# HKUST-Aerial-Robotics/VINS-Mobile

Measured on AMD Instinct MI355X. Metric: VIO frames/sec (KLT+window solve), 640x480/150 feats/W=10, higher is better.
Workload: dtype f64 (solve) / u8+i32+f32 (KLT)

## Files before the change

### include/vio_amd.h

```cpp
#ifndef VIO_AMD_H
#define VIO_AMD_H

#include <stddef.h>
#include <stdint.h>

#ifdef __cplusplus
extern "C" {
#endif

#define VIO_ABI_VERSION 1

#define VIO_OK 0
#define VIO_EINVAL (-1)
#define VIO_ENODEV (-2)
#define VIO_ENOMEM (-3)
#define VIO_ECAP (-4)
#define VIO_ESTATE (-5)
#define VIO_ETIMEOUT (-6)

#define VIO_SIZE_POSE 7
#define VIO_SIZE_SPEEDBIAS 9
#define VIO_MAX_PRIOR_BLOCKS 96

typedef struct VioConfig {
// ... 98 lines not shown
int32_t vio_prior_capacity(int32_t window_size);

typedef struct vio_backend vio_backend_t;

int vio_backend_create(const VioConfig *cfg, int32_t max_batch, vio_backend_t **out);
int vio_backend_get_device(const vio_backend_t *be, int32_t *device);
void vio_backend_destroy(vio_backend_t *be);

int vio_preintegrate(const VioConfig *cfg, const double acc_0[3], const double gyr_0[3],
                     const double ba[3], const double bg[3], int32_t n,
                     const double *dt, const double *acc, const double *gyr,
                     VioPreintegration *out);

int vio_backend_solve_windows(vio_backend_t *be, VioWindow *windows, int32_t n,
                              int32_t buf_num, VioSolveStats *stats );

int vio_backend_reserve_priors(vio_backend_t *be, int32_t n_slots);

int vio_backend_upload(vio_backend_t *be, const VioWindow *windows, int32_t n);
int vio_backend_launch(vio_backend_t *be, void *stream);
int vio_backend_sync(vio_backend_t *be);
int vio_backend_download(vio_backend_t *be, VioWindow *windows, int32_t n, VioSolveStats *stats);
int vio_backend_kernel_ms(vio_backend_t *be, double *ms_avg, int32_t *launches);

#define VIO_N_STAGES 17
int vio_backend_set_profile(vio_backend_t *be, int32_t enable);
int vio_backend_stage_cycles(vio_backend_t *be, int32_t window, int64_t *cycles, int32_t n_stages);

typedef struct vio_frontend vio_frontend_t;

typedef struct VioObs {
  int32_t id;
  double x, y, z;
} VioObs;

typedef struct VioTrackViz {
  float *good_pts;
  double *track_len;
  int32_t cap;
  int32_t n;
} VioTrackViz;

int vio_frontend_create(const VioConfig *cfg, int32_t n_seq, vio_frontend_t **out);
int vio_frontend_get_device(const vio_frontend_t *fe, int32_t *device);
void vio_frontend_destroy(vio_frontend_t *fe);

// ... 469 lines not shown
```

### vins-mobile_amd/abi.py

```python
import ctypes as C
import os

import numpy as np

VIO_OK = 0
VIO_EINVAL, VIO_ENODEV, VIO_ENOMEM, VIO_ECAP, VIO_ESTATE, VIO_ETIMEOUT = -1, -2, -3, -4, -5, -6
VIO_MAX_PRIOR_BLOCKS = 96
VIO_MAX_TRACE = 64
VIO_INIT_BA_MAX_FRAMES = 16
VIO_BLOCK_POSE, VIO_BLOCK_SPEEDBIAS, VIO_BLOCK_EXPOSE = 0, 1, 2
VIO_MARGIN_OLD, VIO_MARGIN_SECOND_NEW, VIO_MARGIN_NONE = 0, 1, 2
STAGES = ["setup_imu", "setup_prior", "eval_prior", "eval_imu", "eval_proj", "scale", "schur", "rhs", "cholesky",
          "tri_solve", "quad_form", "dogleg", "cost_eval", "new2old", "marg_build", "marg_chol", "total",
          "p_zero", "p_fact", "p_gram", "p_feat", "c_potrf", "c_trsm", "imu_raw", "c_wait", "q_w", "backsolve",
          "c_ahead", "tr_vec", "m_prior", "m_imu", "m_fact", "m_gram", "d0", "d1", "d2", "d3", "d4", "d5",
          "v_gd", "v_dot", "v_step", "v_plus", "v_gmax", "v_rest", "b_init", "b_pose", "b_asp", "b_band", "b_gn",
          "e_head", "e_copy", "e_h0dx", "e_tail", "x0", "x1", "x2", "x3"]

_dp = C.POINTER(C.c_double)
_ip = C.POINTER(C.c_int32)


class VioConfig(C.Structure):
    _fields_ = [
# ... 388 lines not shown
    if not os.path.exists(PRODUCT_LIB):
        raise RuntimeError("HIP extension missing: %s (run __graft_entry__.build())" % PRODUCT_LIB)
    lib = C.CDLL(PRODUCT_LIB)
    vp = C.c_void_p
    lib.vio_version.restype = C.c_char_p
    lib.vio_config_default.argtypes = [C.POINTER(VioConfig)]
    lib.vio_prior_capacity.argtypes = [C.c_int32]
    lib.vio_prior_capacity.restype = C.c_int32
    lib.vio_backend_create.argtypes = [C.POINTER(VioConfig), C.c_int32, C.POINTER(vp)]
    lib.vio_backend_destroy.argtypes = [vp]
    lib.vio_backend_destroy.restype = None
    lib.vio_preintegrate.argtypes = [C.POINTER(VioConfig), _dp, _dp, _dp, _dp, C.c_int32, _dp, _dp, _dp,
                                     C.POINTER(VioPreintegration)]
    lib.vio_backend_solve_windows.argtypes = [vp, C.POINTER(VioWindow), C.c_int32, C.c_int32,
                                              C.POINTER(VioSolveStats)]
    lib.vio_backend_reserve_priors.argtypes = [vp, C.c_int32]
    lib.vio_backend_get_device.argtypes = [vp, C.POINTER(C.c_int32)]
    lib.vio_frontend_get_device.argtypes = [vp, C.POINTER(C.c_int32)]
    lib.vio_backend_upload.argtypes = [vp, C.POINTER(VioWindow), C.c_int32]
    lib.vio_backend_launch.argtypes = [vp, vp]
    lib.vio_backend_sync.argtypes = [vp]
    lib.vio_backend_download.argtypes = [vp, C.POINTER(VioWindow), C.c_int32, C.POINTER(VioSolveStats)]
    lib.vio_backend_kernel_ms.argtypes = [vp, _dp, _ip]
    u8p, fp = C.POINTER(C.c_uint8), C.POINTER(C.c_float)
    cfgp = C.POINTER(VioConfig)
    lib.vio_frontend_create.argtypes = [cfgp, C.c_int32, C.POINTER(vp)]
    lib.vio_frontend_destroy.argtypes = [vp]
    lib.vio_frontend_destroy.restype = None
    lib.vio_frontend_read_image.argtypes = [vp, C.c_int32, u8p, C.c_int32, C.c_int32, C.c_int32, C.c_double, C.c_int32,
                                            C.POINTER(VioObs), _ip, vp]
    lib.vio_frontend_read_images.argtypes = [vp, u8p, C.c_int32, C.c_int32, C.c_int32, _dp, C.c_int32,
                                             C.POINTER(VioObs), _ip]
    lib.vio_hip_runtime.argtypes = [C.c_char_p, C.c_int32, _ip]
    lib.vio_host_pool_width.argtypes = [_ip]
    lib.vio_frontend_submit_images.argtypes = [vp, u8p, C.c_int32, C.c_int32, C.c_int32, C.c_int32]
    lib.vio_frontend_submit_images_async.argtypes = [vp, u8p, C.c_int32, C.c_int32, C.c_int32, C.c_int32]
    lib.vio_frontend_collect.argtypes = [vp, C.POINTER(VioObs), _ip]
    lib.vio_host_register.argtypes = [vp, C.c_size_t]
    lib.vio_host_unregister.argtypes = [vp]
    lib.vio_frontend_upload_frames.argtypes = [vp, u8p, C.c_int32, C.c_int32, C.c_int32, C.c_int32]
    lib.vio_frontend_step_resident.argtypes = [vp, C.c_int32, C.c_int32, vp]
    lib.vio_frontend_sync.argtypes = [vp]
    lib.vio_frontend_kernel_ms.argtypes = [vp, _dp, _ip]
    lib.vio_frontend_get_state.argtypes = [vp, C.c_int32, fp, _ip, _ip, C.c_int32, _ip]
    lib.vio_frontend_get_pnp_points.argtypes = [vp, C.c_int32, fp, _ip, C.c_int32, _ip]
    lib.vio_frontend_lk_iterations.argtypes = [vp, C.c_int32, C.POINTER(C.c_uint64), C.POINTER(C.c_uint64), C.c_int32]
# ... 104 lines not shown
```

### vins-mobile_amd/backend.py

```python
import ctypes as C

import numpy as np

from . import abi


class WindowSolver:
    def __init__(self, cfg=None, max_batch=1024):
        self.lib = abi.load_product()
        self.cfg = cfg if cfg is not None else abi.default_config()
        self.max_batch = max_batch
        self._h = C.c_void_p()
        rc = self.lib.vio_backend_create(C.byref(self.cfg), max_batch, C.byref(self._h))
        if rc != abi.VIO_OK:
            raise RuntimeError("vio_backend_create failed rc=%d (a gfx950 device is required)" % rc)
        self._structs = None

    def close(self):
        if self._h:
            self.lib.vio_backend_destroy(self._h)
            self._h = C.c_void_p()

    def __del__(self):
        try:
# ... 3 lines not shown

    def _array(self, windows):
        arr = (abi.VioWindow * len(windows))()
        for i, w in enumerate(windows):
            w.fill_struct(arr[i])
        return arr

    @staticmethod
    def _check(rc, what):
        if rc != abi.VIO_OK:
            raise RuntimeError("%s failed rc=%d" % (what, rc))

    def solve(self, windows, buf_num=0):
        arr = self._array(windows)
        stats = (abi.VioSolveStats * len(windows))()
        self._check(self.lib.vio_backend_solve_windows(self._h, arr, len(windows), buf_num, stats), "solve_windows")
        return [abi.stats_to_dict(s) for s in stats]

    def device(self):
        d = C.c_int32(-1)
        self._check(self.lib.vio_backend_get_device(self._h, C.byref(d)), "get_device")
        return d.value

    def reserve_priors(self, n_slots):
        self._check(self.lib.vio_backend_reserve_priors(self._h, n_slots), "reserve_priors")

    def upload(self, windows):
        self._structs = self._array(windows)
        self._check(self.lib.vio_backend_upload(self._h, self._structs, len(windows)), "upload")

    def launch(self, stream=None):
        self._check(self.lib.vio_backend_launch(self._h, C.c_void_p(stream) if stream else None), "launch")

    def sync(self):
        self._check(self.lib.vio_backend_sync(self._h), "sync")

    def download(self, windows):
        arr = self._array(windows)
        stats = (abi.VioSolveStats * len(windows))()
        self._check(self.lib.vio_backend_download(self._h, arr, len(windows), stats), "download")
        return [abi.stats_to_dict(s) for s in stats]

    def set_profile(self, enable=True):
        self._check(self.lib.vio_backend_set_profile(self._h, 1 if enable else 0), "set_profile")

    def stage_cycles(self, window=0):
# ... 14 lines not shown
```

### vins-mobile_amd/csrc/solver_core.h

```cpp
#pragma once

#include <math.h>
#include <stdint.h>

#include <type_traits>

#include "solve_trace.h"
#include "vio_math.h"

#include "spmd.h"
#include "factors.h"
#include "mfma_tiles.h"

namespace vio {

constexpr int kBS = 15;
constexpr int kSS = kSB * kSB;
constexpr int kAW = 18;
constexpr int kAS = kSB * kAW;

struct WinView {
  int W, P, F, M, np, nblk, has_loop, loop_frame, marg_flag, max_iter;
  int prior_n, prior_nb;
  int Fpad;
// ... 992 lines not shown
  return total;
}


template <class WK>
VIO_DEV double feat_d2(const WK &w, int f) {
  return fmin(fmax(w.sf[f] * w.sf[f] * w.hff[f], 1e-6), 1e32);
}
template <class WK>
VIO_DEV double feat_d(const WK &w, int f) {
  return sqrt_f(feat_d2(w, f));
}
template <class WK>
VIO_DEV double feat_gd(const WK &w, int f) {
  return w.sf[f] * w.gf[f] * rsqrt_f(feat_d2(w, f));
}

template <class WK>
VIO_DEV double pose_gd(const WK &w, int i) {
  return w.sp[i] * w.gp[i] * rcp_f(w.dp[i]);
}

template <class WK>
VIO_DEV double quad_form_H(const Ctx &cx, const WinView &v, WK &w, cldsd vp, cldsd vf, bool prepared = false, bool w_part = true) {
  const int np = v.np, F = v.F, n6 = v.n6, P = v.P;
  if (!prepared) {
    VIO_PARFOR(f, F) w.tf[f] = 0.0;
    VIO_PARFOR(i, np) {
      const int f = i / kBS, c = i - f * kBS;
      const double u = w.sp[i] * vp[i];
      w.t1[i] = u;
      if (c < 6) w.xt[6 * f + c] = u;
    }
    VIO_SYNC();
  }
  int nparts, per;
  wt_parts((int)cx.nt, F, n6, nparts, per);
  if (w_part) VIO_PARFOR(q, F * nparts) {
    const int part = q / F, f = q - part * F;
    const int a0 = part * per, a1 = a0 + per < n6 ? a0 + per : n6;
    double x[kWStrip], sacc = 0;
    for (int b0 = a0; b0 < a1; b0 += kWStrip) {
      const int nb = a1 - b0 < kWStrip ? a1 - b0 : kWStrip;
      wt_strip_load(v.WTf + (size_t)f * v.n6cap + b0, 1, nb, x);
#pragma unroll
      for (int j = 0; j < kWStrip; j++) sacc += (j < nb ? x[j] : 0.0) * w.xt[b0 + (j < nb ? j : 0)];
    }
    VIO_ATOMIC_ADD(w.tf + f, sacc);
  }
  stamp(cx, ST_Q_W);
  double acc = 0;
  VIO_PARFOR(q, 4 * n6) {
    const int r = q >> 2, part = q & 3;
    auto row = w.App + tri_at(r, 0);
    double sacc = 0;
    for (int c = part; c < r; c += 4) sacc = fma(row[c], w.xt[c], sacc);
    sacc *= 2.0;
    if (part == 0) sacc = fma(row[r], w.xt[r], sacc);
    acc = fma(w.xt[r], sacc, acc);
  }
  VIO_PARFOR(q, P * kSB) {
// ... 14 lines not shown
    double s3 = 0, ar[kAW];
#pragma unroll
    for (int jj = 0; jj < kAW; jj++) ar[jj] = A[jj < aw ? jj : 0];
    VIO_SCHED_FENCE();
#pragma unroll
    for (int jj = 0; jj < kAW; jj++) s3 = fma(jj < aw ? ar[jj] : 0.0, w.xt[alo + (jj < aw ? jj : 0)], s3);
    acc = fma(ur, sacc + 2.0 * s3, acc);
  }
  VIO_PARFOR(q, kSB * v.nT) {
    const int c = q / v.nT, j0 = 16 * (q - c * v.nT);
    int kpr = -1;
    for (int k = 0; k < P; k++)
      if (w.sbr[2 * k + 1]) kpr = k;
    if (kpr < 0) continue;
    double xs[16], s3 = 0;
    const double *Ap = v.Apri + (size_t)c * v.jp + j0;
#pragma unroll
    for (int j = 0; j < 16; j++) xs[j] = Ap[j];
    VIO_SCHED_FENCE();
#pragma unroll
    for (int j = 0; j < 16; j++) s3 = fma(xs[j], j0 + j < n6 ? w.xt[j0 + j] : 0.0, s3);
    acc = fma(2.0 * w.t1[kBS * kpr + 6 + c], s3, acc);
  }
  if (w_part) VIO_SYNC();
  VIO_PARFOR(f, F) {
    const double u = w.sf[f] * vf[f];
    acc = fma(u, fma(w.hff[f], u, 2.0 * w.tf[f]), acc);
  }
  return block_sum(cx, acc);
}

template <class FT, class FR>
VIO_DEV void schur_ksplit5(const Ctx &cx, const double *Wf, int ldw, int n6, int F, cldsd einv, cldsd ge, FT flush_tile,
                           FR flush_rhs, cldsd up = nullptr, ldsd tq = nullptr) {
  constexpr int kT = 5;
  const int tid_ = VIO_TID(cx), wave = tid_ >> 6, lane = tid_ & 63, nw = cx.nt >> 6;
  const int li = lane & 15, kq = lane >> 4;
  const int ksteps = (F + 3) / 4;
  const int ksw = (ksteps + nw - 1) / nw;
  const int s_begin = wave * ksw, s_end = s_begin + ksw < ksteps ? s_begin + ksw : ksteps;
  v4d acc[kT * (kT + 1) / 2];
  double rp[kT];
#pragma unroll
  for (int q = 0; q < kT * (kT + 1) / 2; q++) acc[q] = v4d{0.0, 0.0, 0.0, 0.0};
#pragma unroll
  for (int t = 0; t < kT; t++) rp[t] = 0.0;
  double u5[kT];
#pragma unroll
  for (int t = 0; t < kT; t++) u5[t] = (tq && 16 * t + li < n6) ? up[16 * t + li] : 0.0;
  for (int s0 = s_begin; s0 < s_end; s0 += 5) {
    double wv[5][kT], ev[5], gv[5];
#pragma unroll
    for (int j = 0; j < 5; j++) {
      const int f = 4 * (s0 + j) + kq;
      const int fc = (s0 + j < s_end && f < F) ? f : 0;
      ev[j] = einv[fc], gv[j] = ge[fc];
#pragma unroll
      for (int t = 0; t < kT; t++) {
        const int col = 16 * t + li;
        wv[j][t] = Wf[(size_t)fc * ldw + (col < n6 ? col : 0)];
      }
    }
    __builtin_amdgcn_sched_barrier(0);
#pragma unroll
    for (int j = 0; j < 5; j++) {
      const int f = 4 * (s0 + j) + kq;
      const bool vf = s0 + j < s_end && f < F;
#pragma unroll
      for (int t = 0; t < kT; t++) {
        wv[j][t] = (vf && 16 * t + li < n6) ? wv[j][t] : 0.0;
        rp[t] = fma(wv[j][t], gv[j], rp[t]);
      }
      if (tq) {
        double pq = wv[j][0] * u5[0];
#pragma unroll
        for (int t = 1; t < kT; t++) pq = fma(wv[j][t], u5[t], pq);
        pq += dpp_move_f64<0x111, 0xf>(pq);
        pq += dpp_move_f64<0x112, 0xf>(pq);
        pq += dpp_move_f64<0x114, 0xf>(pq);
        pq += dpp_move_f64<0x118, 0xf>(pq);
        if (li == 15 && vf) tq[f] = pq;
      }
#pragma unroll
      for (int ti = 0; ti < kT; ti++) {
        const double a = wv[j][ti] * ev[j];
#pragma unroll
        for (int tj = 0; tj <= ti; tj++) acc[ti * (ti + 1) / 2 + tj] = mfma_f64(a, wv[j][tj], acc[ti * (ti + 1) / 2 + tj]);
      }
    }
  }
#pragma unroll
  for (int ti = 0; ti < kT; ti++)
#pragma unroll
    for (int tj = 0; tj <= ti; tj++) {
      const int bcol = 16 * tj + li;
#pragma unroll
      for (int r = 0; r < 4; r++) {
        const int arow = 16 * ti + kq + 4 * r;
        if (arow < n6 && bcol <= arow) flush_tile(arow, bcol, acc[ti * (ti + 1) / 2 + tj][r]);
      }
    }
#pragma unroll
  for (int t = 0; t < kT; t++) {
    const int a = 16 * t + li;
    if (a < n6 && rp[t] != 0.0) flush_rhs(a, rp[t]);
  }
}

VIO_DEV void schur_add(double *p, double v) { atomic_add_noret(p, v); }
#ifndef VIO_HOST_BUILD
VIO_DEV void schur_add(ldsd p, double v) { atomic_add(p, v); }
#endif

template <class FT, class FR>
VIO_DEV void schur_blocks(const Ctx &cx, const double *Wf, int ldw, int n6, int F, cldsd einv, cldsd ge, int share, int nshare, FT flush_el,
                          FR flush_rhs, cldsd up = nullptr, ldsd tq = nullptr) {
  const int T = (n6 + 15) / 16, NB = (T + 1) / 2, nblocks = NB * (NB + 1) / 2;
  const int tid_ = VIO_TID(cx), wave = tid_ >> 6, lane = tid_ & 63, nw = cx.nt >> 6;
  const int li = lane & 15, kq = lane >> 4;
  const int ksteps = (F + 3) / 4;
  constexpr int kChunk = 6;
  const int nchunks = (ksteps + kChunk - 1) / kChunk;
  int ksplit = 1;
  {
    const int waves = nshare * nw;
    int best = ((nblocks + waves - 1) / waves) * nchunks;
    for (int k = 2; k <= 4; k++) {
      const int cost = ((nblocks * k + waves - 1) / waves) * ((nchunks + k - 1) / k);
      if (cost < best) best = cost, ksplit = k;
    }
  }
  const int ks_part = (nchunks + ksplit - 1) / ksplit * kChunk;
  for (int u = share * nw + wave; u < nblocks * ksplit; u += nshare * nw) {
    const int p = u / ksplit, part = u - p * ksplit;
    const int s_lo = part * ks_part, s_hi = s_lo + ks_part < ksteps ? s_lo + ks_part : ksteps;
    int I = 0;
    while ((I + 1) * (I + 2) / 2 <= p) I++;
    const int J = p - I * (I + 1) / 2;
    const bool diag = I == J;
    const int ta[2] = {2 * I, 2 * I + 1}, tb[2] = {2 * J, 2 * J + 1};
    bool va[2], vb[2];
    const double *pa[2], *pb[2];
#pragma unroll
    for (int q = 0; q < 2; q++) {
      va[q] = ta[q] < T && 16 * ta[q] + li < n6, vb[q] = tb[q] < T && 16 * tb[q] + li < n6;
      pa[q] = Wf + (va[q] ? 16 * ta[q] + li : 0), pb[q] = Wf + (vb[q] ? 16 * tb[q] + li : 0);
    }
    v4d c00 = {0.0, 0.0, 0.0, 0.0}, c01 = c00, c10 = c00, c11 = c00;
    double rp[2] = {0.0, 0.0};
    const bool do_tq = diag && tq != nullptr;
    double u2[2] = {0.0, 0.0};
    if (do_tq) {
#pragma unroll
      for (int q = 0; q < 2; q++) u2[q] = va[q] ? up[16 * ta[q] + li] : 0.0;
    }
    for (int s0 = s_lo; s0 < s_hi; s0 += kChunk) {
      double av[2][kChunk], bv[2][kChunk], ev[kChunk], gv[kChunk];
#pragma unroll
      for (int j = 0; j < kChunk; j++) {
        const int f = 4 * (s0 + j) + kq;
        const size_t fo = (size_t)((f < F && s0 + j < s_hi) ? f : 0) * ldw;
        av[0][j] = pa[0][fo], av[1][j] = pa[1][fo], bv[0][j] = pb[0][fo], bv[1][j] = pb[1][fo];
        ev[j] = einv[(f < F && s0 + j < s_hi) ? f : 0];
        gv[j] = diag ? ge[(f < F && s0 + j < s_hi) ? f : 0] : 0.0;
      }
      VIO_SCHED_FENCE();
#pragma unroll
      for (int j = 0; j < kChunk; j++) {
        const int f = 4 * (s0 + j) + kq;
        const bool vf = f < F && s0 + j < s_hi;
        double pq = 0.0;
#pragma unroll
        for (int q = 0; q < 2; q++) {
          const double a_raw = (va[q] && vf) ? av[q][j] : 0.0;
          if (diag) rp[q] = fma(a_raw, gv[j], rp[q]);
          if (do_tq) pq = fma(a_raw, u2[q], pq);
          av[q][j] = a_raw * ev[j], bv[q][j] = (vb[q] && vf) ? bv[q][j] : 0.0;
        }
        if (do_tq) {
          pq += dpp_move_f64<0x111, 0xf>(pq);
          pq += dpp_move_f64<0x112, 0xf>(pq);
          pq += dpp_move_f64<0x114, 0xf>(pq);
          pq += dpp_move_f64<0x118, 0xf>(pq);
          if (li == 15 && vf) VIO_ATOMIC_ADD(tq + f, pq);
        }
      }
#pragma unroll
      for (int j = 0; j < kChunk; j++) {
        c00 = mfma_f64(av[0][j], bv[0][j], c00), c10 = mfma_f64(av[1][j], bv[0][j], c10), c11 = mfma_f64(av[1][j], bv[1][j], c11);
        if (!diag) c01 = mfma_f64(av[0][j], bv[1][j], c01);
      }
    }
    auto flush = [&](int tr, int tc, const v4d &acc) {
      const int bcol = 16 * tc + li;
#pragma unroll
      for (int r = 0; r < 4; r++) {
        const int arow = 16 * tr + kq + 4 * r;
        if (tr < T && tc < T && arow < n6 && bcol < n6 && bcol <= arow) flush_el(arow, bcol, acc[r], ksplit > 1);
      }
    };
    flush(ta[0], tb[0], c00), flush(ta[1], tb[0], c10), flush(ta[1], tb[1], c11);
    if (!diag) flush(ta[0], tb[1], c01);
    if (diag) {
#pragma unroll
      for (int q = 0; q < 2; q++)
        if (va[q] && rp[q] != 0.0) flush_rhs(16 * ta[q] + li, rp[q]);
    }
  }
}

template <class WK>
VIO_DEV void schur_general(const Ctx &cx, const WinView &v, WK &w, int share, int nshare, ldsd tq = nullptr) {
  const int n6 = v.n6, F = v.F;
  schur_blocks(
      cx, v.WTf, v.n6cap, n6, F, w.einv, w.tf, share, nshare,
      [&](int arow, int bcol, double val, bool parts) {
        if (parts) schur_add(w.App + tri_at(arow, bcol), -val);
        else w.App[tri_at(arow, bcol)] -= val;
      },
      [&](int a, double val) { schur_add(w.App + tri_at(n6, a), -val); },
      w.xt, tq);
  stamp(cx, ST_SCHUR);
}

template <class WK>
VIO_DEV bool build_reduced_system(const Ctx &cx, const WinView &v, WK &w, double mu, ldsd tq = nullptr) {
  const int np = v.np, F = v.F;
  stamp(cx, ST_TR_VEC);
  VIO_PARFOR(f, F) {
    const double isf = rcp_f(w.sf[f]);
    const double e = w.hff[f] + mu * (feat_d2(w, f) * isf * isf);
    const double ei = rcp_f(e);
    w.einv[f] = ei;
    w.tf[f] = w.gf[f] * ei;
    if (!(e > 0.0)) w.flag[0] = 1;
  }
  const bool tq_general = tq != nullptr && ((v.n6 + 15) >> 4) > 5;
  if (tq_general) VIO_PARFOR(f, F) tq[f] = 0.0;
  VIO_PARFOR(i, np) {
    const int f = i / kBS, c = i - f * kBS;
    const double cc = w.dp[i] * rcp_f(w.sp[i]);
    if (c < 6) {
      w.App[tri_at(6 * f + c, 6 * f + c)] += mu * cc * cc;
      w.App[tri_at(v.n6, 6 * f + c)] = w.gp[i];
    } else {
      w.Dss[f * kSS + (c - 6) * (kSB + 1)] += mu * cc * cc;
    }
  }
  VIO_SYNC();
  stamp(cx, ST_SCALE);
  const int n6 = v.n6;
  {
    const int T = (n6 + 15) / 16, npairs = T * (T + 1) / 2;
    const int tid_ = VIO_TID(cx), wave = tid_ >> 6, lane = tid_ & 63, nw = cx.nt >> 6;
    const int li = lane & 15, kq = lane >> 4;
    const int ksteps = (F + 3) / 4;
    constexpr int kT = 5;
    if (T <= kT) {
      schur_ksplit5(cx, v.WTf, v.n6cap, n6, F, w.einv, w.tf,
                    [&](int arow, int bcol, double val) { VIO_ATOMIC_ADD(w.App + tri_at(arow, bcol), -val); },
                    [&](int a, double val) { VIO_ATOMIC_ADD(w.App + tri_at(n6, a), -val); }, w.xt, tq);
    } else {
#ifndef VIO_HOST_BUILD
      if (cx.coop > 1) {
        const CoopLayout L = CoopLayout::make(v.Pcap, v.Fcap, v.nblk_cap);
        VIO_PARFOR(f, F) v.coop[L.o_einv + f] = w.einv[f], v.coop[L.o_tf + f] = w.tf[f];
        if (tq) VIO_PARFOR(q, 16 * T) v.coop[L.o_pose + q] = w.xt[q];
        coop_post(cx, v, COOP_SCHUR);
        schur_general(cx, v, w, 0, cx.coop, tq);
        coop_wait_helpers(cx, v);
        if (tq) {
          VIO_SYNC();
          for (int m = 1; m < cx.coop; m++) {
            const double *pr = v.coop + L.o_part + (size_t)(m - 1) * L.part;
            VIO_PARFOR(f, F) tq[f] += pr[L.p_f + f];
          }
        }
      } else
#endif
        schur_general(cx, v, w, 0, 1, tq);
    }
  }
  VIO_SYNC();
  stamp(cx, ST_RHS);
  (void)np;
  return w.flag[0] == 0;
}


template <class WK>
VIO_DEV void band_step(const Ctx &cx, const WinView &v, WK &w, int k, int fail_flag, int lane_) {
  const int lane = VIO_OPAQUE(lane_), li = lane & 15, kq = lane >> 4;
  ldsd D = w.Dss + k * kSS;
  ldsd ldk = w.ldinv + kSB * k;
  const bool good = potrf9_inv_wave(D, w.Css + (k + 1 <= v.W ? k + 1 : k) * kSS, k < v.W, ldk, lane);
  if (!good && lane == 0) w.flag[fail_flag] = 1;
  stamp(cx, ST_D3);
  if (k >= 1) {
    __builtin_amdgcn_fence(__ATOMIC_RELEASE, "wavefront");
    __builtin_amdgcn_wave_barrier();
    __builtin_amdgcn_fence(__ATOMIC_ACQUIRE, "wavefront");
    ldsd C = w.Css + k * kSS;
    double a[3], b[4];
// ... 936 lines not shown
};

template <bool REGS, int NW, class WK, class VP, class WP>
VIO_DEV void minimize(const Ctx &cx, const WinView &v, WK &w_whole, const VP &fresh, const WP &fresh_work) {
  WK &w = w_whole;
  const int np = v.np, F = v.F;
  const SolveTrace trace{v.stats_d, v.stats_i};
  auto grad_max_norm = [&]() { return gradient_max_norm(cx, fresh(), w); };

  double x_cost = evaluate(cx, fresh(), w, w.xpose, w.xsb, w.xfeat, true, false);
  double x_norm = -1.0;
  VIO_PARFOR(f, F) w.sf[f] = rcp_f(1.0 + sqrt_f(w.hff[f]));
  VIO_SYNC();
  double gmax = grad_max_norm();
  double radius = 1e4, mu = 1e-8;
  const double min_mu = 1e-8, max_mu = 1.0, mu_inc = 10.0;
  bool reuse = false, last_ok = true, have_factor = false;
  double dogleg_step_norm = 0, alpha = 0;
  int it = 0, n_ok = 1, n_bad = 0, invalid_run = 0, termination = 0, recorded = 1;
  StepEvaluator ev = StepEvaluator::at(x_cost);
  double min_rec = x_cost;
  if (cx.tid == 0) trace.record(0, x_cost, radius, 0, 0, gmax, true, true);
  if (cx.tid == 0) trace.initial(x_cost);
  double gd_sq = 0, mu_used = mu, qf_cauchy = 0, qf_part = 0;
  bool qf_pending = false;
  bool relin = false, relin_reuse = false, rec_pending = false;
  int rec_it = 0;
  double rec_step_norm = 0, rec_rho = 0;

  while (true) {
    WK w_iter = fresh_work();
    WK &w = w_iter;
    if (relin) {
      evaluate(cx, fresh(), w, w.xpose, w.xsb, w.xfeat, true, true, relin_reuse);
      if (rec_pending) {
        gmax = grad_max_norm();
        if (cx.tid == 0) trace.record(rec_it, x_cost, radius, rec_step_norm, rec_rho, gmax, true, true);
        stamp(cx, ST_V_GMAX);
      }
      relin = relin_reuse = rec_pending = false;
    }
    if (it >= v.max_iter) break;
    if (last_ok && gmax <= 1e-10) { termination = 1; break; }
    if (radius <= 1e-32) { termination = 1; break; }
    it++;
    bool solver_ok = true;
    if (!reuse) {
      reuse = true;
      ldsd park = w.park;
      if (cx.tid == 0) {
        park[0] = x_cost, park[1] = x_norm, park[2] = gmax, park[3] = radius, park[4] = dogleg_step_norm, park[5] = ev.minimum_cost;
        park[6] = ev.current_cost, park[7] = ev.reference_cost, park[8] = ev.candidate_cost;
        park[9] = ev.accumulated_reference_model_cost_change, park[10] = ev.accumulated_candidate_model_cost_change, park[11] = min_rec;
        ldsi pi = reinterpret_cast<ldsi>(park + 12);
        pi[0] = it, pi[1] = n_ok, pi[2] = n_bad, pi[3] = invalid_run, pi[4] = termination, pi[5] = recorded, pi[6] = last_ok ? 1 : 0;
      }
      {
        double part = 0;
        VIO_PARFOR(i, np) {
          const int f = i / kBS, c = i - f * kBS;
          const double g = pose_gd(w, i), a = g * rcp_f(w.dp[i]), u = w.sp[i] * a;
          part += g * g;
          w.t2[i] = a, w.t1[i] = u;
          if (c < 6) w.xt[6 * f + c] = u;
        }
        VIO_PARFOR(f, F) {
          const double d2 = feat_d2(w, f), sg = w.sf[f] * w.gf[f], g = sg * rsqrt_f(d2);
          part += g * g;
          w.stf[f] = sg * rcp_f(d2), w.tf[f] = 0.0;
        }
        gd_sq = block_sum(cx, part);
      }
      stamp(cx, ST_V_GD);
      const bool fuse_qw = true;
      const double qf_h0 = quad_form_H(cx, fresh(), w, w.t2, w.stf, true, !fuse_qw);
      stamp(cx, ST_QUADFORM);
      solver_ok = false;
      bool first_try = true;
      while (mu < max_mu) {
        if (!first_try) {
          evaluate(cx, fresh(), w, w.xpose, w.xsb, w.xfeat, true, true);
          if (fuse_qw) {
            VIO_PARFOR(i, np) {
              const int f = i / kBS, c = i - f * kBS;
              const double u = w.sp[i] * (pose_gd(w, i) * rcp_f(w.dp[i]));
              w.t1[i] = u;
              if (c < 6) w.xt[6 * f + c] = u;
            }
          }
        }
        first_try = false;
        if (cx.tid == 0) w.flag[0] = 0, w.flag[1] = 0, w.flag[2] = 0, w.flag[3] = 0;
        VIO_PARFOR(k, v.P) w.ready[k] = 0;
        VIO_SYNC();
        bool ok = build_reduced_system(cx, fresh(), w, mu, fuse_qw ? w.cfeat : nullptr);
        if (ok) {
          if constexpr (REGS) ok = factor_band_regs<kPanelTiles, NW>(cx, fresh(), w);
          else ok = factor_band_lds(cx, fresh(), w);
        }
        if (ok) ok = factor_poses(cx, fresh(), w);
        stamp(cx, ST_CHOL);
        if (ok) {
          backsolve(cx, fresh(), w);
          double bad = 0;
          VIO_PARFOR(f, F) {
            double y = (w.tf[f] - w.gnf[f] * w.einv[f]) * rcp_f(w.sf[f]);
            w.gnf[f] = -feat_d(w, f) * y;
            if (!isfinite(y)) bad = 1;
          }
          VIO_PARFOR(i, np) {
            double y = w.t1[i] * rcp_f(w.sp[i]);
            w.gnp[i] = -w.dp[i] * y;
            if (!isfinite(y)) bad = 1;
          }
          if (block_max(cx, bad) > 0) ok = false;
          stamp(cx, ST_TRISOLVE);
        }
        if (ok) { solver_ok = true; mu_used = mu; have_factor = true; break; }
        mu *= mu_inc;
      }
      {
        VIO_SYNC();
        x_cost = park[0], x_norm = park[1], gmax = park[2], radius = park[3], dogleg_step_norm = park[4], ev.minimum_cost = park[5];
        ev.current_cost = park[6], ev.reference_cost = park[7], ev.candidate_cost = park[8];
        ev.accumulated_reference_model_cost_change = park[9], ev.accumulated_candidate_model_cost_change = park[10], min_rec = park[11];
        ldsi pi = reinterpret_cast<ldsi>(park + 12);
        it = pi[0], n_ok = pi[1], n_bad = pi[2], invalid_run = pi[3], termination = pi[4], recorded = pi[5], last_ok = pi[6] != 0;
      }
      if (solver_ok) {
        qf_part = qf_h0, qf_pending = fuse_qw;
        if (!fuse_qw) {
          qf_cauchy = qf_h0 + mu_used * gd_sq;
          alpha = gd_sq / qf_h0;
        }
        stamp(cx, ST_DOGLEG);
      }
    }
    (void)have_factor;
    bool step_valid = false;
    double model_cost_change = 0;
    if (solver_ok) {
      double p1 = 0, p2 = 0, p3 = 0;
      VIO_PARFOR(i, np) p1 += w.gnp[i] * w.gnp[i], p2 += pose_gd(w, i) * w.gnp[i];
      VIO_PARFOR(f, F) {
        p1 += w.gnf[f] * w.gnf[f], p2 += feat_gd(w, f) * w.gnf[f];
        if (qf_pending) p3 += 2.0 * (w.sf[f] * w.sf[f] * w.gf[f] * rcp_f(feat_d2(w, f))) * w.cfeat[f];
      }
      block_sum3(cx, p1, p2, p3);
      stamp(cx, ST_V_DOT);
      if (qf_pending) {
        const double qf_h = qf_part + p3;
        qf_cauchy = qf_h + mu_used * gd_sq;
        alpha = gd_sq / qf_h;
        qf_pending = false;
      }
      double gnn2 = p1, gdot = p2;
      double gradient_norm = sqrt(gd_sq), gauss_newton_norm = sqrt(gnn2);
      double ca, cb;
      bool need_norm = false;
      if (gauss_newton_norm <= radius) {
        ca = 0, cb = 1, dogleg_step_norm = gauss_newton_norm;
      } else if (gradient_norm * alpha >= radius) {
        ca = -(radius / gradient_norm), cb = 0, dogleg_step_norm = radius;
      } else {
        double b_dot_a = -alpha * gdot;
        double a_squared_norm = pow(alpha * gradient_norm, 2.0);
        double b_minus_a_squared_norm = a_squared_norm - 2 * b_dot_a + pow(gauss_newton_norm, 2);
        double c = b_dot_a - a_squared_norm;
        double d = sqrt(c * c + b_minus_a_squared_norm * (pow(radius, 2.0) - a_squared_norm));
        double beta = (c <= 0) ? (d - c) / b_minus_a_squared_norm : (radius * radius - a_squared_norm) / (d + c);
        ca = -alpha * (1.0 - beta), cb = beta;
        need_norm = true;
      }
      VIO_PARFOR(i, np) {
        const double s_ = ca * pose_gd(w, i) + cb * w.gnp[i];
        w.t2[i] = s_ * rcp_f(w.dp[i]) * w.sp[i];
      }
// ... 129 lines not shown
      }
      VIO_PARFOR(q, nFr * 36) w.ppd[q] = 0.0;
      VIO_SYNC();
      VIO_PARFOR(i, nFr + 1) {
        const bool is_ex = i == nFr;
        double R[9];
        if (is_ex) qtoR(Quat{w.ex[3], w.ex[4], w.ex[5], w.ex[6]}, R);
        else qtoR(Quat{w.xpose[7 * i + 3], w.xpose[7 * i + 4], w.xpose[7 * i + 5], w.xpose[7 * i + 6]}, R);
        auto dst = w.rot + 9 * (is_ex ? v.P + 1 : i);
        for (int k = 0; k < 9; k++) dst[k] = R[k];
      }
      VIO_SYNC();
      const double cost = block_sum(cx, projections_jac(cx, v, w, w.xpose, w.xfeat, true, cx.member, cx.coop, false));
      ldsd whv[6] = {w.cfeat, w.stf, w.gnf, w.tf, w.ef, w.einv};
      VIO_PARFOR(q, np) part[L.p_gp + q] = w.gp[q];
      VIO_PARFOR(q, nFr * 36) part[L.p_ppd + q] = w.ppd[q];
      VIO_PARFOR(f, F) {
        part[L.p_f + f] = w.hff[f], part[L.p_f + fs + f] = w.gf[f];
#pragma unroll
        for (int c = 0; c < 6; c++) part[L.p_f + (2 + c) * fs + f] = whv[c][f];
      }
      if (cx.tid == 0) part[L.p_cost] = cost;
    } else if (cmd == COOP_SCHUR) {
      VIO_PARFOR(f, F) w.einv[f] = v.coop[L.o_einv + f], w.tf[f] = v.coop[L.o_tf + f], w.cfeat[f] = 0.0;
      VIO_PARFOR(q, 16 * ((v.n6 + 15) >> 4)) w.xt[q] = v.coop[L.o_pose + q];
      VIO_SYNC();
      schur_general(cx, v, w, cx.member, cx.coop, w.cfeat);
      VIO_SYNC();
      VIO_PARFOR(f, F) part[L.p_f + f] = w.cfeat[f];
    } else if (cmd == COOP_SYRK) {
      band_syrk_share(cx, v, w, cx.member, cx.coop);
    } else {
      break;
    }
    coop_done(cx, v);
  }
}
#endif

template <bool REGS, int NW, class WK, class VP, class WP>
VIO_DEV void solve_window(const Ctx &cx, const WinView &v, WK &w, const VP &fresh, const WP &fresh_work) {
  const int P = v.P, F = v.F;
  VIO_PARFOR(q, P * 7) w.xpose[q] = v.pose0[q];
  VIO_PARFOR(q, P * 9) w.xsb[q] = v.sb0[q];
  VIO_PARFOR(q, F) w.xfeat[q] = v.feat0[q];
  VIO_PARFOR(q, 7) w.ex[q] = v.ex[q];
  if (v.has_loop) VIO_PARFOR(q, 7) w.xpose[7 * P + q] = v.pose0[7 * v.loop_frame + q];
  VIO_PARFOR(q, v.nblk * kBS) w.t1[q] = 0.0, w.t2[q] = 0.0;
  if (cx.tid == 0) w.flag[0] = w.flag[1] = w.flag[2] = w.flag[3] = 0;
  init_band_reach(cx, v, w);
  VIO_SYNC();
  if (cx.prof && cx.tid == cx.prof_tid) {
// ... 71 lines not shown
```

### vins-mobile_amd/csrc/vio_backend.hip

```cpp
#include <hip/hip_runtime.h>

#include <stdio.h>
#include <stdlib.h>

#include <algorithm>
#include <memory>
#include <vector>

#include <chrono>

#include "batch.h"
#include "vio_pool.h"
#include "vio_device.h"
#include "marg_core.h"
#include "vio_window_variants.h"
#include "vio_amd.h"

using namespace vio;

namespace {

using vio_wk::kThreadsGlb;
using vio_wk::kThreadsLds;
constexpr size_t kLdsLimit = vio::kLdsBytes;
// ... 31 lines not shown

struct vio_backend {
  VioConfig cfg;
  std::unique_ptr<vio_resident> res;
  int peers = 2;
  int device = -1;
  int max_batch = 0;
  hipStream_t stream = nullptr;
  LaunchTimer timer;
  int n = 0;
  bool uploaded = false;
  hipStream_t last_stream = nullptr;
  hipEvent_t upload_done = nullptr;
  bool lds_matrix = true;
  int n_lds = 0, n_glb = 0;
  BatchDims d_lds, d_glb;
  size_t lds_bytes_glb = 0;
  DevBuf<int> d_order;
  HostVec<int> h_order;
  bool profile = false;
  size_t lds_bytes = 0;
  int n_cus = 256;
  bool static_w = false;
  bool coop_ok = false;
  DevBuf<long long> d_prof;
  HostBatch hb;
  BatchPtrs B;
  MargPtrs MP;
  DevBuf<unsigned char> d_in;
  DevBuf<int> d_stats_i, d_m_ints;
  DevBuf<double> d_scratch,
      d_hm, d_out_pose, d_out_sb, d_out_feat, d_raw_pose, d_raw_sb, d_raw_feat, d_out_loop, d_stats_d, d_m_x0, d_m_J,
      d_m_r, d_m_scratch;
  int st_n = 0, st_ncap = 0;
  DevBuf<double> d_st_x0[2], d_st_J[2], d_st_r[2];
  std::vector<unsigned char> st_bank;
  std::vector<int> slot_of;
  DevBuf<PriorTab> d_ptab;
  HostVec<PriorTab> h_ptab;
  bool host_prior_in = true, host_prior_out = true, slots_advanced = false;
  HostVec<double> h_out_pose, h_out_sb, h_out_feat, h_raw_pose, h_raw_sb, h_raw_feat, h_out_loop, h_stats_d, h_m_x0,
      h_m_J, h_m_r;
  HostVec<int> h_stats_i, h_m_ints;
  ~vio_backend();
};

// ... 367 lines not shown
  VIO_ON_DEVICE_OF(be);
  hipStream_t st = stream ? (hipStream_t)stream : be->stream;
  if (st != be->stream && be->upload_done) HIP_OK(hipStreamWaitEvent(st, be->upload_done, 0));
  be->last_stream = st;
  if (poison()) {
    HIP_OK(hipMemsetAsync(be->d_scratch.p, 0xff, be->d_scratch.n * sizeof(double), st));
    HIP_OK(hipMemsetAsync(be->d_hm.p, 0xff, be->d_hm.n * sizeof(double), st));
    HIP_OK(hipMemsetAsync(be->d_out_pose.p, 0xff, be->d_out_pose.n * sizeof(double), st));
    HIP_OK(hipMemsetAsync(be->d_stats_d.p, 0xff, be->d_stats_d.n * sizeof(double), st));
    HIP_OK(hipFuncSetAttribute((const void *)poison_lds_kernel, hipFuncAttributeMaxDynamicSharedMemorySize, (int)kLdsLimit));
    hipLaunchKernelGGL(poison_lds_kernel, dim3(2048), dim3(1024), kLdsLimit, st, (int)(kLdsLimit / sizeof(double)));
  }
  {
    const int rct = be->timer.begin(st);
    if (rct != VIO_OK) return rct;
  }
  if (be->n_lds > 0) {
    BatchPtrs Bl = be->B;
    Bl.d = be->d_lds, Bl.order = be->d_order.p;
    int variant = be->d_lds.lds_asp ? 0 : 1;
    if (be->static_w) variant += 3;
    vio_wk::variant(variant, be->MP.prof != nullptr).launch(be->n_lds, be->lds_bytes, st, Bl, be->MP);
  }
  if (be->n_glb > 0) {
    BatchPtrs Bg = be->B;
    Bg.d = be->d_glb, Bg.order = be->d_order.p + be->n_lds;
    int coop = 1;
    if (be->coop_ok && !be->MP.prof && be->lds_bytes_glb > kLdsHalf) {
      const int forced = vio::env_int("VIO_AMD_COOP", 0);
      const int cus = be->n_cus / std::max(1, be->peers);
      const int groups = (be->n_glb + 7) / 8;
      const bool four = groups * 8 * 4 <= cus && (be->d_glb.Wcap >= 24 || groups * 8 * 8 <= cus);
      coop = four ? 4 : groups * 8 * 2 <= cus ? 2 : 1;
      if (forced >= 1 && forced <= vio::kCoopMax && groups * 8 * forced <= cus) coop = forced;
      if (coop > 1) {
        int per_cu = 0;
        if (hipOccupancyMaxActiveBlocksPerMultiprocessor(&per_cu, vio_wk::variant(2, false).fn,
                                                         kThreadsGlb, be->lds_bytes_glb) != hipSuccess ||
            (long long)per_cu * cus < (long long)groups * 8 * coop)
          coop = 1;
      }
    }
    Bg.coop = coop, Bg.n_launch = be->n_glb;
    {
      const int spin = vio::env_int("VIO_AMD_COOP_SPIN", 0);
      Bg.coop_spin = spin > 0 ? (unsigned)spin : vio::kCoopSpinLimit;
      Bg.coop_fault = vio::env_flag("VIO_AMD_COOP_FAULT") ? 1 : 0;
    }
    int grid = be->n_glb;
    if (coop > 1) {
      grid = (be->n_glb + 7) / 8 * 8 * coop;
      HIP_OK(hipMemset2DAsync(be->d_scratch.p + be->B.s.s_coop, be->B.s.scratch * sizeof(double), 0, 32, (size_t)be->B.n, st));
    }
    vio_wk::variant(2, be->MP.prof != nullptr).launch(grid, be->lds_bytes_glb, st, Bg, be->MP);
  }
  HIP_OK(hipGetLastError());
  return be->timer.end(st);
}

int vio_backend_sync(vio_backend_t *be) {
  if (!be) return VIO_EINVAL;
  VIO_ON_DEVICE_OF(be);
  HIP_OK(hipDeviceSynchronize());
  return VIO_OK;
}

int vio_backend_kernel_ms(vio_backend_t *be, double *ms_avg, int32_t *launches) {
  if (!be || !ms_avg || !launches) return VIO_EINVAL;
  VIO_ON_DEVICE_OF(be);
  HIP_OK(hipDeviceSynchronize());
  return be->timer.drain(ms_avg, launches);
}

int vio_backend_set_profile(vio_backend_t *be, int32_t enable) {
  if (!be) return VIO_EINVAL;
  be->profile = enable != 0;
  be->uploaded = false;
  return VIO_OK;
}

int vio_backend_stage_cycles(vio_backend_t *be, int32_t window, int64_t *cycles, int32_t n_stages) {
  if (!be || !cycles || n_stages < 1) return VIO_EINVAL;
  if (!be->uploaded || !be->profile || window < 0 || window >= be->n) return VIO_ESTATE;
  VIO_ON_DEVICE_OF(be);
  HIP_OK(hipDeviceSynchronize());
  long long tmp[ST_COUNT];
  HIP_OK(hipMemcpy(tmp, be->d_prof.p + (size_t)window * ST_COUNT, sizeof(tmp), hipMemcpyDeviceToHost));
  for (int i = 0; i < n_stages; i++) cycles[i] = i < ST_COUNT ? (int64_t)tmp[i] : 0;
  return VIO_OK;
}

static int backend_download_impl(vio_backend_t *be, VioWindow *windows, int32_t n, VioSolveStats *stats);

int vio_backend_download(vio_backend_t *be, VioWindow *windows, int32_t n, VioSolveStats *stats) {
// ... 100 lines not shown
```

Before: 192,100.

## Compute Cauchy quad form lazily only when GN step exceeds radius

Removes the fused accumulation of the H-quadratic-form partials from the Schur complement kernels and the eager gradient/quad-form pass before each solve. Instead, the steepest-descent norm and quad form are computed only when the Gauss-Newton step falls outside the trust region. This path re-evaluates the residuals and stashes and restores the GN step in scratch. It also adds a query for the cooperative launch width. This saves work in the common in-radius case and lightens the Schur inner loops, at the cost of an extra evaluate call when dogleg is needed.

```diff
diff --git a/include/vio_amd.h b/include/vio_amd.h
--- a/include/vio_amd.h
+++ b/include/vio_amd.h
@@ -144,6 +144,7 @@
 int vio_backend_sync(vio_backend_t *be);
 int vio_backend_download(vio_backend_t *be, VioWindow *windows, int32_t n, VioSolveStats *stats);
 int vio_backend_kernel_ms(vio_backend_t *be, double *ms_avg, int32_t *launches);
+int vio_backend_coop_width(const vio_backend_t *be, int32_t *width);
 
 #define VIO_N_STAGES 17
 int vio_backend_set_profile(vio_backend_t *be, int32_t enable);
diff --git a/vins-mobile_amd/abi.py b/vins-mobile_amd/abi.py
--- a/vins-mobile_amd/abi.py
+++ b/vins-mobile_amd/abi.py
@@ -434,6 +434,7 @@
     lib.vio_backend_sync.argtypes = [vp]
     lib.vio_backend_download.argtypes = [vp, C.POINTER(VioWindow), C.c_int32, C.POINTER(VioSolveStats)]
     lib.vio_backend_kernel_ms.argtypes = [vp, _dp, _ip]
+    lib.vio_backend_coop_width.argtypes = [vp, C.POINTER(C.c_int32)]
     u8p, fp = C.POINTER(C.c_uint8), C.POINTER(C.c_float)
     cfgp = C.POINTER(VioConfig)
     lib.vio_frontend_create.argtypes = [cfgp, C.c_int32, C.POINTER(vp)]
diff --git a/vins-mobile_amd/backend.py b/vins-mobile_amd/backend.py
--- a/vins-mobile_amd/backend.py
+++ b/vins-mobile_amd/backend.py
@@ -49,6 +49,11 @@
         self._check(self.lib.vio_backend_get_device(self._h, C.byref(d)), "get_device")
         return d.value
 
+    def coop_width(self):
+        n = C.c_int32(0)
+        self._check(self.lib.vio_backend_coop_width(self._h, C.byref(n)), "coop_width")
+        return n.value
+
     def reserve_priors(self, n_slots):
         self._check(self.lib.vio_backend_reserve_priors(self._h, n_slots), "reserve_priors")
 
diff --git a/vins-mobile_amd/csrc/solver_core.h b/vins-mobile_amd/csrc/solver_core.h
--- a/vins-mobile_amd/csrc/solver_core.h
+++ b/vins-mobile_amd/csrc/solver_core.h
@@ -1038,7 +1038,7 @@
 }
 
 template <class WK>
-VIO_DEV double quad_form_H(const Ctx &cx, const WinView &v, WK &w, cldsd vp, cldsd vf, bool prepared = false, bool w_part = true) {
+VIO_DEV double quad_form_H(const Ctx &cx, const WinView &v, WK &w, cldsd vp, cldsd vf, bool prepared = false) {
   const int np = v.np, F = v.F, n6 = v.n6, P = v.P;
   if (!prepared) {
     VIO_PARFOR(f, F) w.tf[f] = 0.0;
@@ -1052,7 +1052,7 @@
   }
   int nparts, per;
   wt_parts((int)cx.nt, F, n6, nparts, per);
-  if (w_part) VIO_PARFOR(q, F * nparts) {
+  VIO_PARFOR(q, F * nparts) {
     const int part = q / F, f = q - part * F;
     const int a0 = part * per, a1 = a0 + per < n6 ? a0 + per : n6;
     double x[kWStrip], sacc = 0;
@@ -1113,7 +1113,7 @@
     for (int j = 0; j < 16; j++) s3 = fma(xs[j], j0 + j < n6 ? w.xt[j0 + j] : 0.0, s3);
     acc = fma(2.0 * w.t1[kBS * kpr + 6 + c], s3, acc);
   }
-  if (w_part) VIO_SYNC();
+  VIO_SYNC();
   VIO_PARFOR(f, F) {
     const double u = w.sf[f] * vf[f];
     acc = fma(u, fma(w.hff[f], u, 2.0 * w.tf[f]), acc);
@@ -1123,7 +1123,7 @@
 
 template <class FT, class FR>
 VIO_DEV void schur_ksplit5(const Ctx &cx, const double *Wf, int ldw, int n6, int F, cldsd einv, cldsd ge, FT flush_tile,
-                           FR flush_rhs, cldsd up = nullptr, ldsd tq = nullptr) {
+                           FR flush_rhs) {
   constexpr int kT = 5;
   const int tid_ = VIO_TID(cx), wave = tid_ >> 6, lane = tid_ & 63, nw = cx.nt >> 6;
   const int li = lane & 15, kq = lane >> 4;
@@ -1136,9 +1136,6 @@
   for (int q = 0; q < kT * (kT + 1) / 2; q++) acc[q] = v4d{0.0, 0.0, 0.0, 0.0};
 #pragma unroll
   for (int t = 0; t < kT; t++) rp[t] = 0.0;
-  double u5[kT];
-#pragma unroll
-  for (int t = 0; t < kT; t++) u5[t] = (tq && 16 * t + li < n6) ? up[16 * t + li] : 0.0;
   for (int s0 = s_begin; s0 < s_end; s0 += 5) {
     double wv[5][kT], ev[5], gv[5];
 #pragma unroll
@@ -1162,16 +1159,6 @@
         wv[j][t] = (vf && 16 * t + li < n6) ? wv[j][t] : 0.0;
         rp[t] = fma(wv[j][t], gv[j], rp[t]);
       }
-      if (tq) {
-        double pq = wv[j][0] * u5[0];
-#pragma unroll
-        for (int t = 1; t < kT; t++) pq = fma(wv[j][t], u5[t], pq);
-        pq += dpp_move_f64<0x111, 0xf>(pq);
-        pq += dpp_move_f64<0x112, 0xf>(pq);
-        pq += dpp_move_f64<0x114, 0xf>(pq);
-        pq += dpp_move_f64<0x118, 0xf>(pq);
-        if (li == 15 && vf) tq[f] = pq;
-      }
 #pragma unroll
       for (int ti = 0; ti < kT; ti++) {
         const double a = wv[j][ti] * ev[j];
@@ -1205,7 +1192,7 @@
 
 template <class FT, class FR>
 VIO_DEV void schur_blocks(const Ctx &cx, const double *Wf, int ldw, int n6, int F, cldsd einv, cldsd ge, int share, int nshare, FT flush_el,
-                          FR flush_rhs, cldsd up = nullptr, ldsd tq = nullptr) {
+                          FR flush_rhs) {
   const int T = (n6 + 15) / 16, NB = (T + 1) / 2, nblocks = NB * (NB + 1) / 2;
   const int tid_ = VIO_TID(cx), wave = tid_ >> 6, lane = tid_ & 63, nw = cx.nt >> 6;
   const int li = lane & 15, kq = lane >> 4;
@@ -1239,12 +1226,6 @@
     }
     v4d c00 = {0.0, 0.0, 0.0, 0.0}, c01 = c00, c10 = c00, c11 = c00;
     double rp[2] = {0.0, 0.0};
-    const bool do_tq = diag && tq != nullptr;
-    double u2[2] = {0.0, 0.0};
-    if (do_tq) {
-#pragma unroll
-      for (int q = 0; q < 2; q++) u2[q] = va[q] ? up[16 * ta[q] + li] : 0.0;
-    }
     for (int s0 = s_lo; s0 < s_hi; s0 += kChunk) {
       double av[2][kChunk], bv[2][kChunk], ev[kChunk], gv[kChunk];
 #pragma unroll
@@ -1260,20 +1241,11 @@
       for (int j = 0; j < kChunk; j++) {
         const int f = 4 * (s0 + j) + kq;
         const bool vf = f < F && s0 + j < s_hi;
-        double pq = 0.0;
 #pragma unroll
         for (int q = 0; q < 2; q++) {
           const double a_raw = (va[q] && vf) ? av[q][j] : 0.0;
           if (diag) rp[q] = fma(a_raw, gv[j], rp[q]);
-          if (do_tq) pq = fma(a_raw, u2[q], pq);
           av[q][j] = a_raw * ev[j], bv[q][j] = (vb[q] && vf) ? bv[q][j] : 0.0;
-        }
-        if (do_tq) {
-          pq += dpp_move_f64<0x111, 0xf>(pq);
-          pq += dpp_move_f64<0x112, 0xf>(pq);
-          pq += dpp_move_f64<0x114, 0xf>(pq);
-          pq += dpp_move_f64<0x118, 0xf>(pq);
-          if (li == 15 && vf) VIO_ATOMIC_ADD(tq + f, pq);
         }
       }
 #pragma unroll
@@ -1301,7 +1273,7 @@
 }
 
 template <class WK>
-VIO_DEV void schur_general(const Ctx &cx, const WinView &v, WK &w, int share, int nshare, ldsd tq = nullptr) {
+VIO_DEV void schur_general(const Ctx &cx, const WinView &v, WK &w, int share, int nshare) {
   const int n6 = v.n6, F = v.F;
   schur_blocks(
       cx, v.WTf, v.n6cap, n6, F, w.einv, w.tf, share, nshare,
@@ -1309,13 +1281,12 @@
         if (parts) schur_add(w.App + tri_at(arow, bcol), -val);
         else w.App[tri_at(arow, bcol)] -= val;
       },
-      [&](int a, double val) { schur_add(w.App + tri_at(n6, a), -val); },
-      w.xt, tq);
+      [&](int a, double val) { schur_add(w.App + tri_at(n6, a), -val); });
   stamp(cx, ST_SCHUR);
 }
 
 template <class WK>
-VIO_DEV bool build_reduced_system(const Ctx &cx, const WinView &v, WK &w, double mu, ldsd tq = nullptr) {
+VIO_DEV bool build_reduced_system(const Ctx &cx, const WinView &v, WK &w, double mu) {
   const int np = v.np, F = v.F;
   stamp(cx, ST_TR_VEC);
   VIO_PARFOR(f, F) {
@@ -1326,8 +1297,6 @@
     w.tf[f] = w.gf[f] * ei;
     if (!(e > 0.0)) w.flag[0] = 1;
   }
-  const bool tq_general = tq != nullptr && ((v.n6 + 15) >> 4) > 5;
-  if (tq_general) VIO_PARFOR(f, F) tq[f] = 0.0;
   VIO_PARFOR(i, np) {
     const int f = i / kBS, c = i - f * kBS;
     const double cc = w.dp[i] * rcp_f(w.sp[i]);
@@ -1350,26 +1319,18 @@
     if (T <= kT) {
       schur_ksplit5(cx, v.WTf, v.n6cap, n6, F, w.einv, w.tf,
                     [&](int arow, int bcol, double val) { VIO_ATOMIC_ADD(w.App + tri_at(arow, bcol), -val); },
-                    [&](int a, double val) { VIO_ATOMIC_ADD(w.App + tri_at(n6, a), -val); }, w.xt, tq);
+                    [&](int a, double val) { VIO_ATOMIC_ADD(w.App + tri_at(n6, a), -val); });
     } else {
 #ifndef VIO_HOST_BUILD
       if (cx.coop > 1) {
         const CoopLayout L = CoopLayout::make(v.Pcap, v.Fcap, v.nblk_cap);
         VIO_PARFOR(f, F) v.coop[L.o_einv + f] = w.einv[f], v.coop[L.o_tf + f] = w.tf[f];
-        if (tq) VIO_PARFOR(q, 16 * T) v.coop[L.o_pose + q] = w.xt[q];
         coop_post(cx, v, COOP_SCHUR);
-        schur_general(cx, v, w, 0, cx.coop, tq);
+        schur_general(cx, v, w, 0, cx.coop);
         coop_wait_helpers(cx, v);
-        if (tq) {
-          VIO_SYNC();
-          for (int m = 1; m < cx.coop; m++) {
-            const double *pr = v.coop + L.o_part + (size_t)(m - 1) * L.part;
-            VIO_PARFOR(f, F) tq[f] += pr[L.p_f + f];
-          }
-        }
       } else
 #endif
-        schur_general(cx, v, w, 0, 1, tq);
+        schur_general(cx, v, w, 0, 1);
     }
   }
   VIO_SYNC();
@@ -2352,8 +2313,8 @@
   double min_rec = x_cost;
   if (cx.tid == 0) trace.record(0, x_cost, radius, 0, 0, gmax, true, true);
   if (cx.tid == 0) trace.initial(x_cost);
-  double gd_sq = 0, mu_used = mu, qf_cauchy = 0, qf_part = 0;
-  bool qf_pending = false;
+  double gd_sq = 0, mu_used = mu, qf_cauchy = 0;
+  bool cauchy_known = false;
   bool relin = false, relin_reuse = false, rec_pending = false;
   int rec_it = 0;
   double rec_step_norm = 0, rec_rho = 0;
@@ -2385,45 +2346,18 @@
         ldsi pi = reinterpret_cast<ldsi>(park + 12);
         pi[0] = it, pi[1] = n_ok, pi[2] = n_bad, pi[3] = invalid_run, pi[4] = termination, pi[5] = recorded, pi[6] = last_ok ? 1 : 0;
       }
-      {
-        double part = 0;
-        VIO_PARFOR(i, np) {
-          const int f = i / kBS, c = i - f * kBS;
-          const double g = pose_gd(w, i), a = g * rcp_f(w.dp[i]), u = w.sp[i] * a;
-          part += g * g;
-          w.t2[i] = a, w.t1[i] = u;
-          if (c < 6) w.xt[6 * f + c] = u;
-        }
-        VIO_PARFOR(f, F) {
-          const double d2 = feat_d2(w, f), sg = w.sf[f] * w.gf[f], g = sg * rsqrt_f(d2);
-          part += g * g;
-          w.stf[f] = sg * rcp_f(d2), w.tf[f] = 0.0;
-        }
-        gd_sq = block_sum(cx, part);
-      }
-      stamp(cx, ST_V_GD);
-      const bool fuse_qw = true;
-      const double qf_h0 = quad_form_H(cx, fresh(), w, w.t2, w.stf, true, !fuse_qw);
-      stamp(cx, ST_QUADFORM);
+      cauchy_known = false, gd_sq = 0, qf_cauchy = 0, alpha = 0;
       solver_ok = false;
       bool first_try = true;
       while (mu < max_mu) {
         if (!first_try) {
           evaluate(cx, fresh(), w, w.xpose, w.xsb, w.xfeat, true, true);
-          if (fuse_qw) {
-            VIO_PARFOR(i, np) {
-              const int f = i / kBS, c = i - f * kBS;
-              const double u = w.sp[i] * (pose_gd(w, i) * rcp_f(w.dp[i]));
-              w.t1[i] = u;
-              if (c < 6) w.xt[6 * f + c] = u;
-            }
-          }
         }
         first_try = false;
         if (cx.tid == 0) w.flag[0] = 0, w.flag[1] = 0, w.flag[2] = 0, w.flag[3] = 0;
         VIO_PARFOR(k, v.P) w.ready[k] = 0;
         VIO_SYNC();
-        bool ok = build_reduced_system(cx, fresh(), w, mu, fuse_qw ? w.cfeat : nullptr);
+        bool ok = build_reduced_system(cx, fresh(), w, mu);
         if (ok) {
           if constexpr (REGS) ok = factor_band_regs<kPanelTiles, NW>(cx, fresh(), w);
           else ok = factor_band_lds(cx, fresh(), w);
@@ -2457,32 +2391,45 @@
         ldsi pi = reinterpret_cast<ldsi>(park + 12);
         it = pi[0], n_ok = pi[1], n_bad = pi[2], invalid_run = pi[3], termination = pi[4], recorded = pi[5], last_ok = pi[6] != 0;
       }
-      if (solver_ok) {
-        qf_part = qf_h0, qf_pending = fuse_qw;
-        if (!fuse_qw) {
-          qf_cauchy = qf_h0 + mu_used * gd_sq;
-          alpha = gd_sq / qf_h0;
-        }
-        stamp(cx, ST_DOGLEG);
-      }
+      if (solver_ok) stamp(cx, ST_DOGLEG);
     }
     (void)have_factor;
     bool step_valid = false;
     double model_cost_change = 0;
     if (solver_ok) {
-      double p1 = 0, p2 = 0, p3 = 0;
+      double p1 = 0, p2 = 0, dummy3 = 0;
       VIO_PARFOR(i, np) p1 += w.gnp[i] * w.gnp[i], p2 += pose_gd(w, i) * w.gnp[i];
-      VIO_PARFOR(f, F) {
-        p1 += w.gnf[f] * w.gnf[f], p2 += feat_gd(w, f) * w.gnf[f];
-        if (qf_pending) p3 += 2.0 * (w.sf[f] * w.sf[f] * w.gf[f] * rcp_f(feat_d2(w, f))) * w.cfeat[f];
-      }
-      block_sum3(cx, p1, p2, p3);
+      VIO_PARFOR(f, F) p1 += w.gnf[f] * w.gnf[f], p2 += feat_gd(w, f) * w.gnf[f];
+      block_sum3(cx, p1, p2, dummy3);
       stamp(cx, ST_V_DOT);
-      if (qf_pending) {
-        const double qf_h = qf_part + p3;
+      if (!(sqrt(p1) <= radius) && !cauchy_known) {
+        const int nv_ = v.nblk * kBS, o_gnp = 7 * (v.P + 1) + 9 * v.P + F + 2 * nv_, o_gnf = o_gnp + nv_ + 2 * F;
+        VIO_PARFOR(i, np) v.stash[o_gnp + i] = w.gnp[i];
+        VIO_PARFOR(f, F) v.stash[o_gnf + f] = w.gnf[f];
+        evaluate(cx, fresh(), w, w.xpose, w.xsb, w.xfeat, true, true);
+        double part = 0;
+        VIO_PARFOR(i, np) {
+          const int f = i / kBS, c = i - f * kBS;
+          const double g = pose_gd(w, i), a = g * rcp_f(w.dp[i]), u = w.sp[i] * a;
+          part += g * g;
+          w.t2[i] = a, w.t1[i] = u;
+          if (c < 6) w.xt[6 * f + c] = u;
+        }
+        VIO_PARFOR(f, F) {
+          const double d2 = feat_d2(w, f), sg = w.sf[f] * w.gf[f], g = sg * rsqrt_f(d2);
+          part += g * g;
+          w.stf[f] = sg * rcp_f(d2), w.tf[f] = 0.0;
+        }
+        gd_sq = block_sum(cx, part);
+        stamp(cx, ST_V_GD);
+        const double qf_h = quad_form_H(cx, fresh(), w, w.t2, w.stf, true);
         qf_cauchy = qf_h + mu_used * gd_sq;
         alpha = gd_sq / qf_h;
-        qf_pending = false;
+        cauchy_known = true;
+        VIO_PARFOR(i, np) w.gnp[i] = v.stash[o_gnp + i];
+        VIO_PARFOR(f, F) w.gnf[f] = v.stash[o_gnf + f];
+        VIO_SYNC();
+        stamp(cx, ST_QUADFORM);
       }
       double gnn2 = p1, gdot = p2;
       double gradient_norm = sqrt(gd_sq), gauss_newton_norm = sqrt(gnn2);
@@ -2658,12 +2605,9 @@
       }
       if (cx.tid == 0) part[L.p_cost] = cost;
     } else if (cmd == COOP_SCHUR) {
-      VIO_PARFOR(f, F) w.einv[f] = v.coop[L.o_einv + f], w.tf[f] = v.coop[L.o_tf + f], w.cfeat[f] = 0.0;
-      VIO_PARFOR(q, 16 * ((v.n6 + 15) >> 4)) w.xt[q] = v.coop[L.o_pose + q];
+      VIO_PARFOR(f, F) w.einv[f] = v.coop[L.o_einv + f], w.tf[f] = v.coop[L.o_tf + f];
       VIO_SYNC();
-      schur_general(cx, v, w, cx.member, cx.coop, w.cfeat);
-      VIO_SYNC();
-      VIO_PARFOR(f, F) part[L.p_f + f] = w.cfeat[f];
+      schur_general(cx, v, w, cx.member, cx.coop);
     } else if (cmd == COOP_SYRK) {
       band_syrk_share(cx, v, w, cx.member, cx.coop);
     } else {
diff --git a/vins-mobile_amd/csrc/vio_backend.hip b/vins-mobile_amd/csrc/vio_backend.hip
--- a/vins-mobile_amd/csrc/vio_backend.hip
+++ b/vins-mobile_amd/csrc/vio_backend.hip
@@ -77,6 +77,7 @@
   size_t lds_bytes = 0;
   int n_cus = 256;
   bool static_w = false;
+  int coop_width = 1;
   bool coop_ok = false;
   DevBuf<long long> d_prof;
   HostBatch hb;
@@ -490,6 +491,7 @@
     if (be->static_w) variant += 3;
     vio_wk::variant(variant, be->MP.prof != nullptr).launch(be->n_lds, be->lds_bytes, st, Bl, be->MP);
   }
+  be->coop_width = 1;
   if (be->n_glb > 0) {
     BatchPtrs Bg = be->B;
     Bg.d = be->d_glb, Bg.order = be->d_order.p + be->n_lds;
@@ -510,6 +512,7 @@
       }
     }
     Bg.coop = coop, Bg.n_launch = be->n_glb;
+    be->coop_width = coop;
     {
       const int spin = vio::env_int("VIO_AMD_COOP_SPIN", 0);
       Bg.coop_spin = spin > 0 ? (unsigned)spin : vio::kCoopSpinLimit;
@@ -538,6 +541,12 @@
   VIO_ON_DEVICE_OF(be);
   HIP_OK(hipDeviceSynchronize());
   return be->timer.drain(ms_avg, launches);
+}
+
+int vio_backend_coop_width(const vio_backend_t *be, int32_t *width) {
+  if (!be || !width) return VIO_EINVAL;
+  *width = be->coop_width;
+  return VIO_OK;
 }
 
 int vio_backend_set_profile(vio_backend_t *be, int32_t enable) {
```

Measured after the change: 196,900, median of 6. 2.5% higher.
